# COMBINE-lab/salmon

Measured on NVIDIA H100. Metric: EM iters/s, higher is better.
Workload: dtype f64

## Files before the change

include/salmon_b200.h:

```cpp
#ifndef SALMON_B200_H
#define SALMON_B200_H

#include <stddef.h>
#include <stdint.h>

#ifdef __cplusplus
extern "C" {
#endif

#define SB_OK 0
#define SB_ERR_INVALID (-1)
#define SB_ERR_NO_DEVICE (-2)
#define SB_ERR_CUDA (-3)
#define SB_ERR_NOMEM (-4)
#define SB_ERR_NCCL (-5)
#define SB_ERR_STATE (-6)

int sb_version(void);
const char* sb_last_error(void);
int sb_device_count(void);

typedef struct sb_eq_csr {
  uint64_t n_classes;
  uint32_t n_txps;
// ... 341 lines not shown
                     sb_map_batch_stats* stats);

typedef struct sb_read_meta {
  const char* names;
  const uint64_t* name_off;
  const uint8_t* qual_left;
  const uint8_t* qual_right;
} sb_read_meta;
int64_t sb_reads_next_meta(sb_reads* r, uint32_t max_pairs, uint32_t stride, uint8_t* left, uint8_t* right,
                           uint32_t* len_left, uint32_t* len_right, int want_quals, sb_read_meta* meta);
typedef int (*sb_batch_meta_cb)(void* user, const uint8_t* left, const uint8_t* right, uint32_t n_pairs, uint32_t read_len,
                                const sb_read_meta* meta);
typedef void (*sb_names_cb)(void* user, const char* names, size_t len);
int sb_reads_bucketed_meta(sb_reads* rd, uint32_t min_len, uint32_t batch, uint32_t max_read_len, uint32_t threads,
                           uint32_t shard_index, uint32_t shard_count, int want_quals, sb_batch_meta_cb cb,
                           sb_names_cb too_short, void* user, sb_bucket_stats* stats);

int sb_em_debug_timeline(sb_em_ctx* ctx, uint64_t* out, uint32_t iteration);

int sb_em_set_option(sb_em_ctx* ctx, const char* key, int64_t value);

int sb_em_get_info(sb_em_ctx* ctx, const char* key, int64_t* value);

int sb_nccl_unique_id(void* out128);
int sb_em_comm_init(sb_em_ctx* ctx, int rank, int nranks, const void* unique_id128);
int sb_em_comm_destroy(sb_em_ctx* ctx);
int sb_em_peer_handle(sb_em_ctx* ctx, uint32_t max_txps, void* out64);
int sb_em_peer_open(sb_em_ctx* ctx, int rank, int nranks, const void* handles );

int sb_flush_l2(sb_em_ctx* ctx);

int sb_host_register(void* ptr, size_t bytes);
int sb_host_unregister(void* ptr);

#ifdef __cplusplus
}
#endif
#endif
```

salmon_b200/_capi.py:

```python
from __future__ import annotations

import ctypes as C
import os
from dataclasses import dataclass

import numpy as np

_HERE = os.path.dirname(os.path.abspath(__file__))
LIB_PATH = os.path.join(_HERE, "libsalmon_b200.so")

SB_OK = 0


class SalmonB200Error(RuntimeError):
    pass


class sb_eq_csr(C.Structure):
    _fields_ = [
        ("n_classes", C.c_uint64),
        ("n_txps", C.c_uint32),
        ("off", C.c_void_p),
        ("tids", C.c_void_p),
        ("weights", C.c_void_p),
# ... 152 lines not shown
    "sb_eq_file_read": (C.c_int, [C.c_char_p, C.POINTER(C.POINTER(sb_eq_file))]),
    "sb_eq_file_free": (None, [C.POINTER(sb_eq_file)]),
    "sb_bootstrap_writer_open": (_P, [C.c_char_p]),
    "sb_bootstrap_writer_write": (C.c_int, [_P, _P, C.c_uint32]),
    "sb_bootstrap_writer_close": (C.c_int64, [_P]),
    "sb_txome_read_fasta": (C.c_int, [C.c_char_p, C.c_uint32, C.c_int, C.c_char_p, C.c_int, C.c_int,
                                      C.POINTER(C.POINTER(sb_txome))]),
    "sb_txome_free": (None, [C.POINTER(sb_txome)]),
    "sb_version": (C.c_int, []),
    "sb_last_error": (C.c_char_p, []),
    "sb_device_count": (C.c_int, []),
    "sb_em_default_params": (None, [C.POINTER(sb_em_params)]),
    "sb_em_create": (_P, [C.c_int]),
    "sb_em_destroy": (None, [_P]),
    "sb_em_optimize": (C.c_int, [_P, C.POINTER(sb_eq_csr), C.POINTER(sb_em_params), _P, _P, _P, _P,
                                 C.POINTER(sb_em_stats)]),
    "sb_em_upload": (C.c_int, [_P, C.POINTER(sb_eq_csr), _P, _P, _P]),
    "sb_em_prepare": (C.c_int, [_P, C.POINTER(sb_em_params), C.POINTER(sb_em_stats)]),
    "sb_em_run": (C.c_int, [_P, C.POINTER(sb_em_stats)]),
    "sb_em_download": (C.c_int, [_P, _P, C.POINTER(sb_em_stats)]),
    "sb_em_get_combined": (C.c_int, [_P, _P, _P]),
    "sb_em_set_option": (C.c_int, [_P, C.c_char_p, C.c_int64]),
    "sb_em_get_info": (C.c_int, [_P, C.c_char_p, C.POINTER(C.c_int64)]),
    "sb_em_debug_timeline": (C.c_int, [_P, _P, C.c_uint32]),
    "sb_bootstrap": (C.c_int, [_P, C.POINTER(sb_em_params), C.c_double, C.c_uint32, C.c_uint64, _P, _P]),
    "sb_bootstrap_last_counts": (C.c_int, [_P, _P]),
    "sb_gibbs": (C.c_int, [_P, _P, C.c_int, C.c_int, C.c_double, C.c_uint32, C.c_uint32, C.c_int, C.c_double,
                           C.c_uint64, _P, _P]),
    "sb_gibbs_last_state": (C.c_int, [_P, _P, _P]),
    "sb_nccl_unique_id": (C.c_int, [_P]),
    "sb_em_comm_init": (C.c_int, [_P, C.c_int, C.c_int, _P]),
    "sb_em_comm_destroy": (C.c_int, [_P]),
    "sb_em_peer_handle": (C.c_int, [_P, C.c_uint32, _P]),
    "sb_em_peer_open": (C.c_int, [_P, C.c_int, C.c_int, _P]),
    "sb_flush_l2": (C.c_int, [_P]),
    "sb_index_build": (_P, [C.c_uint32, _P, _P, C.c_uint32]),
    "sb_index_free": (None, [_P]),
    "sb_index_set_meta": (C.c_int, [_P, _P, _P, C.c_uint32]),
    "sb_index_get_meta": (C.c_int, [_P, _P, _P, _P, _P, _P]),
    "sb_index_save": (C.c_int, [_P, C.c_char_p]),
    "sb_index_load": (_P, [C.c_char_p]),
    "sb_index_info": (C.c_int, [_P, _P]),
    "sb_index_host_arrays": (C.c_int, [_P, _P, _P, _P, _P, _P, _P]),
    "sb_map_default_params": (None, [C.POINTER(sb_map_params)]),
    "sb_map_mimic_bt2": (C.c_int, [C.POINTER(sb_map_params), C.c_int]),
    "sb_map_create": (_P, [_P, C.POINTER(sb_map_params), C.c_int, C.c_uint32, C.c_uint32]),
# ... 161 lines not shown
            raise SalmonB200Error("sb_em_create failed: " + self.lib.sb_last_error().decode())
        self._keep = None
        self.M = 0

    def close(self):
        if self.h:
            self.lib.sb_em_destroy(self.h)
            self.h = None

    def __del__(self):
        try:
            self.close()
        except Exception:
            pass

    def set_option(self, key: str, value: int):
        _check(self.lib.sb_em_set_option(self.h, key.encode(), int(value)), "sb_em_set_option")

    def info(self, key: str) -> int:
        v = C.c_int64(0)
        _check(self.lib.sb_em_get_info(self.h, key.encode(), C.byref(v)), "sb_em_get_info")
        return v.value

    @staticmethod
    def _txp_arrays(eq, projected, eff_len, unique):
        projected = np.ascontiguousarray(projected, dtype=np.float64)
        eff_len = np.ascontiguousarray(eff_len, dtype=np.float64)
        unique = np.ascontiguousarray(unique, dtype=np.uint64)
        assert projected.shape[0] == eff_len.shape[0] == unique.shape[0] == eq.n_txps
        return projected, eff_len, unique

    def optimize(self, eq: EqClasses, params: sb_em_params, projected, eff_len, unique):
        projected, eff_len, unique = self._txp_arrays(eq, projected, eff_len, unique)
        alpha = np.empty(eq.n_txps, dtype=np.float64)
        st = sb_em_stats()
        s = eq.as_struct()
        rc = _check(self.lib.sb_em_optimize(self.h, C.byref(s), C.byref(params), projected.ctypes.data,
                                            eff_len.ctypes.data, unique.ctypes.data, alpha.ctypes.data,
                                            C.byref(st)), "sb_em_optimize")
        self.M = eq.n_txps
        self._nnz = eq.nnz
        self._C = eq.n_classes
        return alpha, st, rc == 0

    def upload(self, eq: EqClasses, projected, eff_len, unique):
        projected, eff_len, unique = self._txp_arrays(eq, projected, eff_len, unique)
# ... 669 lines not shown
```

salmon_b200/csrc/em.cu:

```cuda
#include <cooperative_groups.h>
#include <cub/cub.cuh>
#include <float.h>
#include <math.h>
#include <stdarg.h>
#include <string.h>

#include <algorithm>
#include <string>
#include <vector>

#include "common.cuh"
#include "em_internal.h"

#include "em_kernels.cuh"

namespace sb {

static const void* const K_PERSISTENT[2] = {(const void*)k_em_persistent<false>, (const void*)k_em_persistent<true>};
static const void* const K_PERSISTENT_MGPU[2] = {(const void*)k_em_persistent_mgpu<false>,
                                                 (const void*)k_em_persistent_mgpu<true>};
static void (*const K_P1[2])(EmArgs) = {k_em_p1<false>, k_em_p1<true>};
static void (*const K_P2[2])(EmArgs, uint32_t) = {k_em_p2<false>, k_em_p2<true>};
static void (*const K_P2_PARTIAL[2])(EmArgs) = {k_em_p2_partial<false>, k_em_p2_partial<true>};

// ... 153 lines not shown
  const uint32_t t = rank_tid[rowperm[r]];
  row_tid[r] = t;
  tid_row[t] = r;
  r_prior[r] = prior[t];
  r_base[r] = base[t];
  r_alpha0[r] = alpha0[t];
}
__global__ void k_gather_csc(uint32_t nnz, const uint32_t* __restrict__ perm,
                             const uint32_t* __restrict__ ent_cls,
                             const double* __restrict__ m_w, uint32_t* __restrict__ t_idx,
                             double* __restrict__ t_w) {
  uint32_t k = blockIdx.x * blockDim.x + threadIdx.x;
  if (k >= nnz) return;
  uint32_t j = perm[k];
  t_idx[k] = ent_cls[j];
  t_w[k] = m_w[j];
}
__global__ void k_remap(uint32_t n, const uint32_t* __restrict__ src,
                        const uint32_t* __restrict__ map, uint32_t* __restrict__ dst) {
  uint32_t k = blockIdx.x * blockDim.x + threadIdx.x;
  if (k < n) dst[k] = map[src[k]];
}

__global__ void k_sell_widths(uint32_t n_rows, uint32_t n_slices, const uint32_t* __restrict__ rowperm,
                              const uint32_t* __restrict__ csr_off, const uint32_t* __restrict__ csr_idx,
                              uint16_t* __restrict__ len16, uint32_t* __restrict__ width,
                              uint32_t* __restrict__ sbase, uint32_t* __restrict__ counts) {
  const uint32_t s = blockIdx.x * (blockDim.x >> 5) + (threadIdx.x >> 5);
  if (s >= n_slices) return;
  const uint32_t lane = threadIdx.x & 31;
  const uint32_t row = s * 32 + lane;
  uint32_t len = 0, lo = 0xffffffffu, hi = 0;
  bool sell = false;
  if (row < n_rows) {
    const uint32_t cr = rowperm ? rowperm[row] : row;
    const uint32_t b = csr_off[cr];
    len = csr_off[cr + 1] - b;
    sell = len <= LMAX;
    if (!sell) {
      len16[row] = LEN_LONG;
      atomicAdd(&counts[0], 1u);
      len = 0;
    }
    for (uint32_t j = 0; j < len; ++j) {
      lo = min(lo, csr_idx[b + j]);
      hi = max(hi, csr_idx[b + j]);
// ... 11 lines not shown
    if (fallback) {
      atomicAdd(&counts[0], 1u);
      atomicAdd(&counts[2], 1u);
    }
  }
  if (lane == 0) {
    width[s] = fallback ? 0u : width_s;
    sbase[s] = hi >= lo ? lo : 0u;
  }
}
__global__ void k_sell_fill(uint32_t n_rows, uint32_t n_slices, const uint32_t* __restrict__ rowperm,
                            const uint32_t* __restrict__ csr_off, const uint32_t* __restrict__ csr_idx,
                            const double* __restrict__ csr_w, const uint32_t* __restrict__ slice_ptr,
                            const uint32_t* __restrict__ sbase, const uint16_t* __restrict__ len16,
                            uint16_t* __restrict__ s_idx, double* __restrict__ s_w,
                            uint32_t* __restrict__ long_rows, uint32_t* __restrict__ long_cursor) {
  const uint32_t s = blockIdx.x * (blockDim.x >> 5) + (threadIdx.x >> 5);
  if (s >= n_slices) return;
  const uint32_t lane = threadIdx.x & 31;
  const uint32_t row = s * 32 + lane;
  const size_t first = (size_t)slice_ptr[s] * 32;
  const uint32_t width = slice_ptr[s + 1] - slice_ptr[s];
  const uint32_t grouped = width & ~3u;
  auto pos = [&](uint32_t j) {
    return j < grouped ? first + (size_t)(j >> 2) * 128 + lane * 4 + (j & 3u) : first + (size_t)j * 32 + lane;
  };
  const uint32_t base = sbase[s];
  uint32_t n = 0;
  if (row < n_rows) {
    const uint32_t cr = rowperm ? rowperm[row] : row;
    const uint32_t b = csr_off[cr], e = csr_off[cr + 1];
    if (len16[row] == LEN_LONG) {
      const uint32_t pos = atomicAdd(long_cursor, 1u);
      long_rows[3 * pos] = row;
      long_rows[3 * pos + 1] = b;
      long_rows[3 * pos + 2] = e;
    } else {
      n = e - b;
      for (uint32_t j = 0; j < n; ++j) {
        s_idx[pos(j)] = (uint16_t)(csr_idx[b + j] - base);
        s_w[pos(j)] = csr_w[b + j];
      }
    }
  }
  for (uint32_t j = n; j < width; ++j) {
    s_idx[pos(j)] = IDX_PAD;
    s_w[pos(j)] = 0.0;
  }
}
__global__ void k_warp_ranges(uint32_t n_slices, const uint32_t* __restrict__ slice_ptr,
                              uint32_t overhead, uint32_t n_warps, uint32_t* __restrict__ warp_begin) {
  const uint32_t wid = blockIdx.x * blockDim.x + threadIdx.x;
  if (wid > n_warps) return;
  if (wid == n_warps || n_slices == 0) { warp_begin[wid] = n_slices; return; }
  const uint64_t total = (uint64_t)slice_ptr[n_slices] + (uint64_t)overhead * n_slices;
  const uint64_t target = total * wid / n_warps;
  uint32_t lo = 0, hi = n_slices;
  while (lo < hi) {
    uint32_t mid = (lo + hi) >> 1;
    uint64_t wk = (uint64_t)slice_ptr[mid] + (uint64_t)overhead * mid;
    if (wk >= target) hi = mid; else lo = mid + 1;
  }
  warp_begin[wid] = lo;
}

__global__ void k_sum1(uint32_t M, const double* __restrict__ a, const double* __restrict__ b,
                       const uint32_t* __restrict__ tid_row, int mode, double* __restrict__ out) {
  __shared__ double scratch[32];
  double acc = 0.0;
  for (uint32_t i = threadIdx.x; i < M; i += blockDim.x) {
    if (mode == 1 && tid_row[i] != 0xffffffffu) continue;
    acc += a[i] + b[i];
// ... 212 lines not shown
  else if (!strcmp(key, "sample_offset")) { c->sample_offset = (uint32_t)value; }
  else if (!strcmp(key, "rebalance")) { c->rebalance = (int)value; c->prepared = false; }
  else { set_error("unknown option '%s'", key); return SB_ERR_INVALID; }
  return SB_OK;
}

extern "C" int sb_em_get_info(sb_em_ctx* c, const char* key, int64_t* value) {
  if (!c || !key || !value) { set_error("null argument"); return SB_ERR_INVALID; }
  if (!c->prepared) { set_error("sb_em_get_info before sb_em_prepare"); return SB_ERR_STATE; }
  auto stream = [](const SellDev& m) { return (int64_t)m.n_cols * 32 * 10 + (int64_t)m.long_entries * 12; };
  if (!strcmp(key, "stream_bytes")) { *value = stream(c->cm) + stream(c->tm); return SB_OK; }
  if (!strcmp(key, "warps")) { *value = (int64_t)c->grid * (EM_THREADS / 32); return SB_OK; }
  if (!strcmp(key, "ring_cols")) { *value = (int64_t)EM_CH * EM_RING; return SB_OK; }
  const size_t n = strlen(key);
  const SellDev* m = nullptr;
  if (n > 3 && !strcmp(key + n - 3, "_cm")) m = &c->cm;
  else if (n > 3 && !strcmp(key + n - 3, "_tm")) m = &c->tm;
  const std::string k(key, m ? n - 3 : n);
  if (m && k == "stream_bytes") *value = stream(*m);
  else if (m && k == "sell_cols") *value = m->n_cols;
  else if (m && k == "long_rows") *value = m->n_long;
  else if (m && k == "long_entries") *value = (int64_t)m->long_entries;
  else if (m && k == "fallback_rows") *value = m->n_fallback;
  else { set_error("unknown info key '%s'", key); return SB_ERR_INVALID; }
  return SB_OK;
}

extern "C" int sb_em_upload(sb_em_ctx* c, const sb_eq_csr* eq, const double* projected,
                            const double* eff_len, const uint64_t* unique) {
  if (!c || !eq || !projected || !eff_len || !unique) { set_error("null argument"); return SB_ERR_INVALID; }
  if (eq->n_classes && (!eq->off || !eq->counts)) { set_error("null CSR arrays"); return SB_ERR_INVALID; }
  SB_CUDA(cudaSetDevice(c->device));
  const uint64_t C = eq->n_classes;
  const uint32_t M = eq->n_txps;
  const uint64_t nnz = C ? eq->off[C] : 0;
  if (M == 0) { set_error("no transcripts"); return SB_ERR_INVALID; }
  if (nnz >= 0xfffffff0ull || C >= 0xfffffff0ull) {
    set_error("eq-class table too large for 32-bit device offsets (nnz=%llu)", (unsigned long long)nnz);
    return SB_ERR_INVALID;
  }
  if (nnz && (!eq->tids || !eq->weights)) { set_error("null CSR arrays"); return SB_ERR_INVALID; }
  c->C = C; c->M = M; c->nnz = nnz;
  c->prepared = false;
  SB_TRY(dev_alloc(&c->d_off, C + 1));
  SB_TRY(dev_alloc(&c->d_tids, nnz));
  SB_TRY(dev_alloc(&c->d_aux, nnz));
  SB_TRY(dev_alloc(&c->d_counts, C));
// ... 100 lines not shown
  }
  m.n_block = 0;
  m.long_entries = 0;
  if (m.n_long > 0) {
    std::vector<uint32_t> h((size_t)3 * m.n_long);
    SB_CUDA(cudaMemcpyAsync(h.data(), m.long_rows, h.size() * 4, cudaMemcpyDeviceToHost, st));
    SB_CUDA(cudaStreamSynchronize(st));
    std::vector<uint32_t> ord(m.n_long);
    for (uint32_t i = 0; i < m.n_long; ++i) ord[i] = i;
    std::sort(ord.begin(), ord.end(), [&](uint32_t x, uint32_t y) {
      const uint32_t lx = h[3 * x + 2] - h[3 * x + 1], ly = h[3 * y + 2] - h[3 * y + 1];
      return lx != ly ? lx > ly : h[3 * x] < h[3 * y];
    });
    for (uint32_t i = 0; i < m.n_long; ++i) {
      if (h[3 * ord[i] + 2] - h[3 * ord[i] + 1] > LWARP) m.n_block = i + 1;
      m.long_entries += h[3 * i + 2] - h[3 * i + 1];
    }
    std::vector<uint32_t> h2(h.size());
    for (uint32_t i = 0; i < m.n_long; ++i)
      for (int k = 0; k < 3; ++k) h2[3 * i + k] = h[3 * ord[i] + k];
    SB_CUDA(cudaMemcpyAsync(m.long_rows, h2.data(), h2.size() * 4, cudaMemcpyHostToDevice, st));
    SB_CUDA(cudaStreamSynchronize(st));
  }
  k_warp_ranges<<<nblk(n_warps + 1, 256), 256, 0, st>>>(m.n_slices, m.slice_ptr, overhead, n_warps, m.warp_begin);
  c->launches++;
  return SB_OK;
}

static int em_rebalance(sb_em_ctx* c);

extern "C" int sb_em_prepare(sb_em_ctx* c, const sb_em_params* p, sb_em_stats* stats) {
  if (!c || !p) { set_error("null argument"); return SB_ERR_INVALID; }
  if (!c->uploaded) { set_error("sb_em_prepare before sb_em_upload"); return SB_ERR_STATE; }
  SB_CUDA(cudaSetDevice(c->device));
  cudaStream_t st = c->stream;
  c->params = *p;
  c->launches = 0;
  const uint64_t C = c->C;
  const uint32_t M = c->M;
  const uint64_t nnz = c->nnz;
  const bool row_space = c->nranks <= 1 && !c->fused_loopback;
  SB_CUDA(cudaEventRecord(c->ev[0], st));

  int occ = 0;
  for (int v = 0; v < 2; ++v) {
    SB_CUDA(cudaFuncSetAttribute(K_PERSISTENT[v], cudaFuncAttributeMaxDynamicSharedMemorySize, (int)EM_SMEM));
    SB_CUDA(cudaFuncSetAttribute((const void*)K_P1[v], cudaFuncAttributeMaxDynamicSharedMemorySize, (int)EM_SMEM));
    SB_CUDA(cudaFuncSetAttribute((const void*)K_P2[v], cudaFuncAttributeMaxDynamicSharedMemorySize, (int)EM_SMEM));
// ... 190 lines not shown
    stats->gpu_launches = prep_launches;
  }
  return SB_OK;
}

static Sell sell_view(const SellDev& m) {
  Sell s;
  s.slice_ptr = m.slice_ptr; s.base = m.base; s.len = m.len; s.idx = m.idx; s.w = m.w; s.warp_begin = m.warp_begin;
  s.long_rows = m.long_rows; s.csr_idx = m.csr_idx; s.csr_w = m.csr_w;
  s.n_rows = m.n_rows; s.n_slices = m.n_slices; s.n_long = m.n_long;
  s.n_block = m.n_block;
  s.zero = m.zero;
  return s;
}

static void fill_args(sb_em_ctx* c, EmArgs& A, bool row_space) {
  memset(&A, 0, sizeof(A));
  A.cm = sell_view(c->cm);
  A.tm = sell_view(c->tm);
  const bool ov = c->ov_active;
  A.c_cnt = (ov && c->ov_cnt) ? c->ov_cnt : c->d_cnt; A.scale = c->d_scale;
  if (row_space) {
    A.alpha = c->r_alpha; A.theta = c->r_theta; A.prior = c->r_prior;
    A.base = (ov && c->ov_base_row) ? c->ov_base_row : c->r_base;
    A.row_tid = nullptr;
  } else {
    A.alpha = c->d_alpha; A.theta = c->d_theta; A.prior = c->d_prior; A.base = c->d_base;
    A.row_tid = c->d_row_tid;
    A.tid_row = c->d_tid_row;
  }
  A.sum_partial = c->d_sum_partial;
  A.maxrel = (unsigned long long*)(c->d_scalars + 24);
  A.inactive_sum = ov ? c->ov_inactive_sum : c->inactive_sum;
  A.sum0 = ov ? c->ov_sum0 : c->sum0;
  A.min_eq_w = ov ? c->ov_min_eq_w : DBL_MIN;
  A.first_bias = ov ? 0.0 : (c->params.use_vbem ? 0.0 : 1.0);
  A.tol = c->params.tol; A.min_iter = c->params.min_iter; A.max_iter = c->params.max_iter;
  A.out = (uint32_t*)(c->d_scalars + 32);
  A.lq = (unsigned int*)(c->d_scalars + 44);
  A.dbg = c->dbg_enabled ? c->d_dbg : nullptr;
  A.dbg_it = c->dbg_it;
}

#include <dlfcn.h>
namespace {
struct NcclUid { char b[128]; };
// ... 524 lines not shown
```

salmon_b200/csrc/em_internal.h:

```cpp
#pragma once
#include <cuda_runtime.h>
#include <stdint.h>

#include <vector>

#include "../../include/salmon_b200.h"

namespace sb {

constexpr int SELL_GROUP = 1024;

struct SellDev {
  uint32_t n_rows = 0, n_slices = 0, n_cols = 0, n_long = 0, n_block = 0;
  uint32_t n_fallback = 0;
  uint64_t long_entries = 0;
  uint32_t zero = 0;
  uint32_t* slice_ptr = nullptr;
  uint32_t* width = nullptr;
  uint32_t* base = nullptr;
  uint16_t* len = nullptr;
  uint16_t* idx = nullptr;
  double* w = nullptr;
  uint32_t* warp_begin = nullptr;
  uint32_t* long_rows = nullptr;
  const uint32_t* csr_idx = nullptr;
  const double* csr_w = nullptr;
};

}

struct sb_em_ctx {
  int device = 0;
  int n_sm = 0;
  size_t l2_bytes = 0;
  cudaStream_t stream = nullptr;
  cudaEvent_t ev[4] = {nullptr, nullptr, nullptr, nullptr};

  int variant = 1;
// ... 103 lines not shown
```

salmon_b200/csrc/em_kernels.cuh:

```cuda
#pragma once
#include <cooperative_groups.h>
#include <float.h>

#include "common.cuh"
#include "em_math.h"

namespace sb {
namespace cg = cooperative_groups;

constexpr uint32_t LMAX = 96;
constexpr uint32_t LWARP = 2048;
constexpr int EM_THREADS = 256;
constexpr int EM_CH = 8;
constexpr int EM_RING = 4;
constexpr int EM_MIN_BLOCKS = 2;
constexpr double DIGAMMA_MIN = 1e-10;
constexpr double MIN_EQ_W = DBL_MIN;
constexpr double ALPHA_CHECK_CUTOFF = 1e-2;
constexpr uint16_t LEN_LONG = 0xFFFFu;
constexpr uint16_t IDX_PAD = 0xFFFFu;
constexpr uint32_t DBG_ACCUMULATE = 0xFFFFFFFFu;
constexpr uint32_t DBG_SLOTS = 16;

struct Sell {
  const uint32_t* slice_ptr;
  const uint32_t* base;
  const uint16_t* len;
  const uint16_t* idx;
  const double* w;
  const uint32_t* warp_begin;
  const uint32_t* long_rows;
  const uint32_t* csr_idx;
  const double* csr_w;
  uint32_t n_rows, n_slices, n_long;
  uint32_t n_block;
  uint32_t zero;
};

struct EmArgs {
  Sell cm;
  Sell tm;
  const double* c_cnt;
  double* scale;
  double* alpha; double* theta; const double* prior; const double* base;
  const uint32_t* row_tid;
  const uint32_t* tid_row;
  double* part_out;
  double* sum_partial;
  unsigned long long* maxrel;
  double inactive_sum; double sum0;
  double tol;
  double min_eq_w;
  double first_bias;
  uint32_t min_iter, max_iter;
  uint32_t* out;
  unsigned long long* dbg;
  uint32_t dbg_it;
  unsigned int* lq;
  unsigned char* const* peers;
  uint32_t rank, nranks, M;
  uint32_t push_pass;
  unsigned long long epoch0;
  uint32_t* xfail;
};

constexpr uint32_t XAUX = 1024;
struct XchgLayout {
  uint32_t M, G, S;
  __host__ __device__ XchgLayout(uint32_t m, uint32_t g) : M(m), G(g), S((m + g - 1) / g) {}
  __host__ __device__ size_t off_flags() const { return 0; }
  __host__ __device__ size_t off_theta() const { return 64 * 8; }
  __host__ __device__ size_t off_alpha() const { return off_theta() + ((size_t)M + 4) * 8; }
  __host__ __device__ size_t off_llth() const { return (off_alpha() + (size_t)M * 8 + 15) & ~(size_t)15; }
  __host__ __device__ size_t off_llaux() const { return off_llth() + (size_t)M * 16; }
  __host__ __device__ size_t off_llrecv() const { return off_llaux() + (size_t)G * XAUX * 2 * 16; }
  __host__ __device__ size_t bytes() const { return off_llrecv() + (size_t)G * S * 16; }
};

__device__ __forceinline__ unsigned long long gtime_ns() {
  unsigned long long t;
  asm volatile("mov.u64 %0, %%globaltimer;" : "=l"(t));
  return t;
}

constexpr double SUM_FIXED = 1048576.0;
struct P2Acc {
  long long isum;
  double maxrel;
};
__device__ __forceinline__ long long warp_sum_ll(long long v) {
#pragma unroll
  for (int o = 16; o > 0; o >>= 1) v += __shfl_xor_sync(0xffffffffu, v, o);
  return v;
}
__device__ __forceinline__ long long block_sum_ll(long long v, double* scratch) {
  const int lane = threadIdx.x & 31, wid = threadIdx.x >> 5;
  const int nw = (blockDim.x + 31) >> 5;
  v = warp_sum_ll(v);
  __syncthreads();
  if (lane == 0) scratch[wid] = __longlong_as_double(v);
  __syncthreads();
  long long r = (lane < nw) ? __double_as_longlong(scratch[lane]) : 0ll;
  return warp_sum_ll(r);
}

struct __align__(128) WarpRing {
  double w[EM_RING][EM_CH * 32];
  uint16_t idx[EM_RING][EM_CH * 32];
};
constexpr int EM_WARPS = EM_THREADS / 32;
constexpr size_t EM_SMEM = sizeof(WarpRing) * EM_WARPS + EM_WARPS * EM_RING * 8 + 40 * 8;
// ... 12 lines not shown
__device__ __forceinline__ void warp_setup(WarpCtx& W, unsigned char* smem) {
  const uint32_t wid = threadIdx.x >> 5;
  W.ring = reinterpret_cast<WarpRing*>(smem) + wid;
  W.bars = reinterpret_cast<uint64_t*>(smem + sizeof(WarpRing) * EM_WARPS) + wid * EM_RING;
  W.scratch = reinterpret_cast<double*>(smem + sizeof(WarpRing) * EM_WARPS + EM_WARPS * EM_RING * 8);
  W.phase_bits = 0;
  W.dbg = nullptr;
  W.dbg_acc = nullptr;
  W.t0 = 0;
  W.pol_stream = l2_policy_evict_first();
  if ((threadIdx.x & 31u) == 0) {
#pragma unroll
    for (int s = 0; s < EM_RING; ++s) mbar_init(&W.bars[s], 1);
    mbar_fence_init();
  }
  __syncthreads();
}

struct RowOps {
  double x0, x1, x2, x3;
  uint32_t len;
};
template <int PHASE>
__device__ __forceinline__ RowOps load_ops(const EmArgs& A, const Sell& S, uint32_t row) {
  RowOps o;
  o.x0 = o.x1 = o.x2 = o.x3 = 0.0;
  o.len = LEN_LONG;
  if (row < S.n_rows) {
    o.len = __ldg(&S.len[row]);
    if (PHASE == 1) {
      o.x0 = __ldg(&A.c_cnt[row]);
    } else if (PHASE == 2) {
      o.x0 = A.theta[row];
      o.x1 = __ldg(&A.prior[row]);
      o.x2 = __ldg(&A.base[row]);
      o.x3 = A.alpha[row];
    } else {
      const uint32_t t = __ldg(&A.row_tid[row]);
      o.x0 = A.theta[t];
      o.x2 = __ldg(&A.base[t]);
      o.x3 = __longlong_as_double((long long)t);
    }
  }
  return o;
}

template <bool VBEM>
__device__ __forceinline__ double theta_of(double na, double ap, double logNorm) {
  if (VBEM) return (ap > DIGAMMA_MIN) ? exp_digamma_shifted(ap, logNorm) : 0.0;
  return na;
}

template <int PHASE, bool VBEM, class Deliver>
__device__ __forceinline__ void row_finish(const EmArgs& A, uint32_t row, const RowOps& o, double acc,
                                           double logNorm, double bias, P2Acc& pa, Deliver&& deliver) {
  if (o.len == LEN_LONG) return;
  if (PHASE == 1) {
    A.scale[row] = (acc <= A.min_eq_w) ? 0.0 : o.x0 / acc;
  } else if (PHASE == 2) {
    const double th = o.x0, pr = o.x1;
    double na = o.x2 + bias;
    if (th > 0.0) na = fma(th, acc, na);
    if (na > ALPHA_CHECK_CUTOFF) pa.maxrel = fmax(pa.maxrel, fabs(o.x3 - na) / na);
    A.alpha[row] = na;
    const double ap = na + pr;
    pa.isum += __double2ll_rn(ap * SUM_FIXED);
    A.theta[row] = theta_of<VBEM>(na, ap, logNorm);
  } else {
    const uint32_t t = (uint32_t)__double_as_longlong(o.x3);
    double na = o.x2;
    if (o.x0 > 0.0) na = fma(o.x0, acc, na);
    deliver(t, na);
  }
}

struct WarpRange {
  uint32_t s0, s1, cbeg, cend;
};
__device__ __forceinline__ WarpRange load_range(const Sell& S, uint32_t gwarp) {
  WarpRange r;
  r.s0 = __ldg(&S.warp_begin[gwarp]);
  r.s1 = __ldg(&S.warp_begin[gwarp + 1]);
  r.cbeg = __ldg(&S.slice_ptr[r.s0]);
  r.cend = __ldg(&S.slice_ptr[r.s1]);
  return r;
}
__device__ __forceinline__ void ring_issue(const Sell& S, WarpCtx& W, const WarpRange& R, uint32_t k) {
// ... 68 lines not shown
  };
  struct Group {
    double g0, g1, g2, g3;
    double2 wa, wb;
  };
  auto group_load = [&](uint32_t c, uint32_t base) {
    const uint2 i2 = cols.idx4(c);
    Group q;
    q.g0 = gsrc[slot(base, i2.x & 0xFFFFu)];
    q.g1 = gsrc[slot(base, i2.x >> 16)];
    q.g2 = gsrc[slot(base, i2.y & 0xFFFFu)];
    q.g3 = gsrc[slot(base, i2.y >> 16)];
    q.wa = cols.w4(c, 0u);
    q.wb = cols.w4(c, 2u);
    return q;
  };
  auto group_fma = [&](double& acc, const Group& q) {
    fma1(acc, q.g0, q.wa.x); fma1(acc, q.g1, q.wa.y); fma1(acc, q.g2, q.wb.x); fma1(acc, q.g3, q.wb.y);
  };
  uint32_t sbase = s0;
  uint32_t sp = (s0 + lane < s1) ? __ldg(&S.slice_ptr[s0 + lane + 1]) : cend;
  uint32_t sb = (s0 + lane < s1) ? __ldg(&S.base[s0 + lane]) : 0u;
  uint32_t c = 0;
  RowOps ops_next = load_ops<PHASE>(A, S, s0 * 32u + lane);
  for (uint32_t s = s0; s < s1; ++s) {
    if (s - sbase == 32u) {
      sbase = s;
      sp = (s + lane < s1) ? __ldg(&S.slice_ptr[s + lane + 1]) : cend;
      sb = (s + lane < s1) ? __ldg(&S.base[s + lane]) : 0u;
    }
    const uint32_t slice_end = __shfl_sync(0xffffffffu, sp, (int)(s - sbase)) - cbeg;
    const uint32_t base = __shfl_sync(0xffffffffu, sb, (int)(s - sbase));
    uint32_t ng = (slice_end - c) >> 2;
    const uint32_t rem = (slice_end - c) & 3u;
    const RowOps ops = ops_next;
    if (s + 1u < s1) ops_next = load_ops<PHASE>(A, S, (s + 1u) * 32u + lane);
    if (slice_end == c) continue;
    double acc = 0.0;
    for (; ng >= 2; ng -= 2, c += 8) {
      cols.need(c, c + 8);
      const Group qa = group_load(c, base);
      const Group qb = group_load(c + 4, base);
      group_fma(acc, qa);
      group_fma(acc, qb);
    }
    if (ng) {
      cols.need(c, c + 4);
      group_fma(acc, group_load(c, base));
      c += 4;
    }
    if (rem) {
      cols.need(c, c + rem);
      const double g0 = gsrc[slot(base, cols.idx1(c))];
      if (rem == 1) {
        fma1(acc, g0, cols.w1(c));
      } else if (rem == 2) {
        const double g1 = gsrc[slot(base, cols.idx1(c + 1))];
        fma1(acc, g0, cols.w1(c)); fma1(acc, g1, cols.w1(c + 1));
      } else {
// ... 32 lines not shown
    const uint32_t r = __ldg(&S.long_rows[3 * li]);
    const uint32_t b = __ldg(&S.long_rows[3 * li + 1]);
    const uint32_t e = __ldg(&S.long_rows[3 * li + 2]);
    double a0 = 0.0, a1 = 0.0;
    uint32_t k = b + threadIdx.x;
    for (; k + EM_THREADS < e; k += 2 * EM_THREADS) {
      const uint32_t i0 = __ldg(&S.csr_idx[k]), i1 = __ldg(&S.csr_idx[k + EM_THREADS]);
      double v0 = gsrc[i0] * __ldg(&S.csr_w[k]);
      double v1 = gsrc[i1] * __ldg(&S.csr_w[k + EM_THREADS]);
      if (GUARD) {
        if (isnan(v0)) v0 = 0.0;
        if (isnan(v1)) v1 = 0.0;
      }
      a0 += v0;
      a1 += v1;
    }
    if (k < e) {
      double v = gsrc[__ldg(&S.csr_idx[k])] * __ldg(&S.csr_w[k]);
      if (GUARD && isnan(v)) v = 0.0;
      a0 += v;
    }
    const double acc = block_reduce<false>(a0 + a1, W.scratch);
    if (threadIdx.x == 0) {
      RowOps o = load_ops<PHASE>(A, S, r);
      o.len = 0;
      row_finish<PHASE, VBEM>(A, r, o, acc, logNorm, bias, pa, deliver);
    }
    __syncthreads();
  }
  {
    const uint32_t gw = bid * EM_WARPS + (threadIdx.x >> 5);
    const uint32_t nw = nblk * EM_WARPS;
    const uint32_t n_mid = S.n_long - S.n_block;
    unsigned int* queue = A.lq + ((PHASE == 1) ? 0 : 1);
    uint32_t cnt = 0, myrow = 0xffffffffu;
    double myacc = 0.0;
    auto flush = [&]() {
      if (myrow != 0xffffffffu) {
        RowOps o = load_ops<PHASE>(A, S, myrow);
        o.len = 0;
        row_finish<PHASE, VBEM>(A, myrow, o, myacc, logNorm, bias, pa, deliver);
      }
      myrow = 0xffffffffu;
      cnt = 0;
    };
    auto claim = [&]() -> uint32_t {
      uint32_t q = 0;
      if (lane == 0) q = atomicAdd(queue, 1u);
      return q;
    };
    uint32_t q_next;
    if (DYNQ) q_next = n_mid ? claim() : 0u; else q_next = gw;
    unsigned long long* const qs = (dbg && lane == 0) ? dbg + (PHASE == 1 ? 9 : 11) : nullptr;
    for (;;) {
      const uint32_t q = DYNQ ? __shfl_sync(0xffffffffu, q_next, 0) : q_next;
      if (q >= n_mid) break;
      if (DYNQ) q_next = claim(); else q_next = q + nw;
      const uint32_t li = S.n_block + q;
      const uint32_t r = __ldg(&S.long_rows[3 * li]);
      const uint32_t b = __ldg(&S.long_rows[3 * li + 1]);
      const uint32_t e = __ldg(&S.long_rows[3 * li + 2]);
      double a0 = 0.0, a1 = 0.0, a2 = 0.0, a3 = 0.0;
// ... 93 lines not shown
  W.dbg_acc = nullptr; \
  if (dbg_acc && (threadIdx.x & 31u) == 0) A.dbg[(size_t)gwarp * DBG_SLOTS + (slot)] += gtime_ns() - var;

template <bool VBEM>
__global__ void __launch_bounds__(EM_THREADS, EM_MIN_BLOCKS) k_em_persistent(const __grid_constant__ EmArgs A) {
  extern __shared__ __align__(128) unsigned char smem[];
  WarpCtx W;
  warp_setup(W, smem);
  double* scratch = W.scratch;
  cg::grid_group grid = cg::this_grid();
  const uint32_t bid = blockIdx.x, nblk = gridDim.x;
  const uint32_t gwarp = bid * (EM_THREADS / 32) + (threadIdx.x >> 5);
  const WarpRange R1 = load_range(A.cm, gwarp);
  const WarpRange R2 = load_range(A.tm, gwarp);
  uint32_t it = 0;
  bool converged = false;
  double logNorm = VBEM ? digamma_pos(A.sum0) : 0.0;
  ring_prefetch(A.cm, W, R1);
  while (it < A.min_iter || (it < A.max_iter && !converged)) {
    const uint32_t par = it & 1u;
    const bool dbg_acc = A.dbg && A.dbg_it == DBG_ACCUMULATE && it > 0;
    if (bid == 0 && threadIdx.x == 0) A.maxrel[par] = 0ull;
    if (VBEM && it > 0) lag_lognorm_warp0(A, par, nblk, scratch);
    P2Acc pa{0ll, 0.0};
    SB_DBG(0)
    SB_ACC_BEGIN(t1, 3)
    W.dbg = (A.dbg && it == A.dbg_it) ? &A.dbg[(size_t)gwarp * DBG_SLOTS] : nullptr;
    run_phase<1, VBEM, true>(A, W, R1, bid, nblk, 0.0, 0.0, pa, [&] { ring_prefetch(A.tm, W, R2); }, NoDeliver{});
    SB_ACC_END(t1, 0)
    SB_DBG(1)
    grid.sync();
    SB_DBG(2)
    if (bid == 0 && threadIdx.x == 0) A.lq[0] = 0u;
    if (VBEM && it > 0) logNorm = scratch[33];
    const double bias = (it == 0) ? A.first_bias : 0.0;
    SB_DBG(3)
    SB_ACC_BEGIN(t2, 4)
    run_phase<2, VBEM, true>(A, W, R2, bid, nblk, logNorm, bias, pa, [&] { ring_prefetch(A.cm, W, R1); }, NoDeliver{});
    W.dbg = nullptr;
    SB_ACC_END(t2, 1)
    SB_DBG(4)
    p2_finish(A, scratch, pa, par);
    SB_DBG(5)
    grid.sync();
    SB_DBG(6)
    if (bid == 0 && threadIdx.x == 0) A.lq[1] = 0u;
    if (dbg_acc && (threadIdx.x & 31u) == 0) A.dbg[(size_t)gwarp * DBG_SLOTS + 2] += 1ull;
// ... 90 lines not shown
  cg::grid_group grid = cg::this_grid();
  const uint32_t bid = blockIdx.x, nblk = gridDim.x;
  const uint32_t gwarp = bid * (EM_THREADS / 32) + (threadIdx.x >> 5);
  const uint32_t gtid = bid * EM_THREADS + threadIdx.x, gthreads = nblk * EM_THREADS;
  const WarpRange R1 = load_range(A.cm, gwarp);
  const WarpRange R2 = load_range(A.tm, gwarp);
  const uint32_t M = A.M, G = A.nranks;
  const XchgLayout X(M, G);
  const uint32_t S = X.S, lo = min(A.rank * S, M), hi = min(lo + S, M);
  unsigned char* const own = A.peers[A.rank];
  const uint4* my_recv = reinterpret_cast<const uint4*>(own + X.off_llrecv());
  const uint4* my_llth = reinterpret_cast<const uint4*>(own + X.off_llth());
  const uint4* my_aux = reinterpret_cast<const uint4*>(own + X.off_llaux());
  double* theta = A.theta;
  uint32_t it = 0;
  bool converged = false;
  double logNorm = VBEM ? digamma_pos(A.sum0) : 0.0;
  ring_prefetch(A.cm, W, R1);
  while (it < A.min_iter || (it < A.max_iter && !converged)) {
    const uint32_t par = it & 1u;
    const uint32_t epoch = (uint32_t)(A.epoch0 + it + 1ull);
    const DeliverPush push{A.peers, X.off_llrecv(), S, A.rank, epoch};
    const bool dbg_acc = A.dbg && A.dbg_it == DBG_ACCUMULATE && it > 0;
    P2Acc pa{0ll, 0.0};
    SB_DBG(0)
    SB_ACC_BEGIN(t1, 3)
    run_phase<1, VBEM, true>(A, W, R1, bid, nblk, 0.0, 0.0, pa, [&] { ring_prefetch(A.tm, W, R2); }, NoDeliver{});
    SB_ACC_END(t1, 0)
    SB_DBG(1)
    grid.sync();
    SB_DBG(2)
    if (bid == 0 && threadIdx.x == 0) A.lq[0] = 0u;
    SB_ACC_BEGIN(t2, 4)
    if (A.push_pass) {
      run_phase<3, VBEM, true>(A, W, R2, bid, nblk, 0.0, 0.0, pa, [&] { ring_prefetch(A.cm, W, R1); },
                               DeliverLocal{A.part_out});
      SB_ACC_END(t2, 1)
      SB_DBG(3)
      __threadfence();
      grid.sync();
      if (bid == 0 && threadIdx.x == 0) A.lq[1] = 0u;
      for (uint32_t t = gtid; t < M; t += gthreads) push(t, __ldcg(&A.part_out[t]));
    } else {
      for (uint32_t t = gtid; t < M; t += gthreads)
        if (__ldg(&A.tid_row[t]) == 0xffffffffu) push(t, __ldg(&A.base[t]));
      run_phase<3, VBEM, true>(A, W, R2, bid, nblk, 0.0, 0.0, pa, [&] { ring_prefetch(A.cm, W, R1); }, push);
      SB_ACC_END(t2, 1)
// ... 89 lines not shown
    SB_DBG(7)
    if (dbg_acc && (threadIdx.x & 31u) == 0) A.dbg[(size_t)gwarp * DBG_SLOTS + 2] += 1ull;
    ++it;
  }
  for (uint32_t t = lo + gtid; t < hi; t += gthreads) {
    const double a = A.alpha[t];
    for (uint32_t q = 0; q < G; ++q) st_relaxed_sys_f64(reinterpret_cast<double*>(A.peers[q] + X.off_alpha()) + t, a);
  }
  xgpu_barrier(grid, A, A.epoch0 + it + 1ull);
  if (bid == 0 && threadIdx.x == 0) {
    A.out[0] = it;
    A.out[1] = converged ? 1u : 0u;
    A.out[2] = (it - 1) & 1u;
    A.out[3] = it + 2u;
  }
  ring_drain(W, R1);
}

template <bool VBEM>
__global__ void __launch_bounds__(EM_THREADS, EM_MIN_BLOCKS) k_em_p1(const __grid_constant__ EmArgs A) {
  extern __shared__ __align__(128) unsigned char smem[];
  WarpCtx W;
  warp_setup(W, smem);
  P2Acc pa{0ll, 0.0};
  const WarpRange R = load_range(A.cm, blockIdx.x * (EM_THREADS / 32) + (threadIdx.x >> 5));
  ring_prefetch(A.cm, W, R);
  run_phase<1, VBEM, false>(A, W, R, blockIdx.x, gridDim.x, 0.0, 0.0, pa, Nothing{}, NoDeliver{});
}
template <bool VBEM>
__global__ void __launch_bounds__(EM_THREADS, EM_MIN_BLOCKS) k_em_p2(const __grid_constant__ EmArgs A, uint32_t it) {
  extern __shared__ __align__(128) unsigned char smem[];
  WarpCtx W;
  warp_setup(W, smem);
  double* scratch = W.scratch;
  const uint32_t par = it & 1u;
  double logNorm = 0.0;
  if (VBEM) {
    if (it == 0) {
      logNorm = digamma_pos(A.sum0);
    } else {
      lag_lognorm_warp0(A, par, gridDim.x, scratch);
      __syncthreads();
      logNorm = scratch[33];
    }
  }
  const double bias = (it == 0) ? A.first_bias : 0.0;
  P2Acc pa{0ll, 0.0};
  const WarpRange R = load_range(A.tm, blockIdx.x * (EM_THREADS / 32) + (threadIdx.x >> 5));
  ring_prefetch(A.tm, W, R);
  run_phase<2, VBEM, false>(A, W, R, blockIdx.x, gridDim.x, logNorm, bias, pa, Nothing{}, NoDeliver{});
  p2_finish(A, scratch, pa, par);
}
template <bool VBEM>
__global__ void __launch_bounds__(EM_THREADS, EM_MIN_BLOCKS) k_em_p2_partial(const __grid_constant__ EmArgs A) {
  extern __shared__ __align__(128) unsigned char smem[];
  WarpCtx W;
  warp_setup(W, smem);
  P2Acc pa{0ll, 0.0};
  const WarpRange R = load_range(A.tm, blockIdx.x * (EM_THREADS / 32) + (threadIdx.x >> 5));
  ring_prefetch(A.tm, W, R);
  run_phase<3, VBEM, false>(A, W, R, blockIdx.x, gridDim.x, 0.0, 0.0, pa, Nothing{}, DeliverLocal{A.part_out});
}

}
```

Baseline: 26710.

## Skip alpha reads/writes before min_iter and broadcast uniform prior

```diff
diff --git a/include/salmon_b200.h b/include/salmon_b200.h
--- a/include/salmon_b200.h
+++ b/include/salmon_b200.h
@@ -387,6 +387,9 @@
 
 int sb_em_get_info(sb_em_ctx* ctx, const char* key, int64_t* value);
 
+int sb_em_get_layout(sb_em_ctx* ctx, int which, uint32_t* slice_ptr, uint32_t* base, uint16_t* idx,
+                     uint32_t* long_rows, uint32_t* csr_idx);
+
 int sb_nccl_unique_id(void* out128);
 int sb_em_comm_init(sb_em_ctx* ctx, int rank, int nranks, const void* unique_id128);
 int sb_em_comm_destroy(sb_em_ctx* ctx);
diff --git a/salmon_b200/_capi.py b/salmon_b200/_capi.py
--- a/salmon_b200/_capi.py
+++ b/salmon_b200/_capi.py
@@ -198,6 +198,7 @@
     "sb_em_get_combined": (C.c_int, [_P, _P, _P]),
     "sb_em_set_option": (C.c_int, [_P, C.c_char_p, C.c_int64]),
     "sb_em_get_info": (C.c_int, [_P, C.c_char_p, C.POINTER(C.c_int64)]),
+    "sb_em_get_layout": (C.c_int, [_P, C.c_int, _P, _P, _P, _P, _P]),
     "sb_em_debug_timeline": (C.c_int, [_P, _P, C.c_uint32]),
     "sb_bootstrap": (C.c_int, [_P, C.POINTER(sb_em_params), C.c_double, C.c_uint32, C.c_uint64, _P, _P]),
     "sb_bootstrap_last_counts": (C.c_int, [_P, _P]),
@@ -405,6 +406,16 @@
         _check(self.lib.sb_em_get_info(self.h, key.encode(), C.byref(v)), "sb_em_get_info")
         return v.value
 
+    def layout(self, which: str, rows: int, nnz_multi: int) -> dict:
+        ns = (rows + 31) // 32
+        out = {"slice_ptr": np.zeros(ns + 1, np.uint32), "base": np.zeros(max(ns, 1), np.uint32),
+               "idx": np.zeros(max(self.info("sell_cols_" + which) * 32, 1), np.uint16),
+               "long_rows": np.zeros(max(3 * self.info("long_rows_" + which), 1), np.uint32),
+               "csr_idx": np.zeros(max(nnz_multi, 1), np.uint32)}
+        _check(self.lib.sb_em_get_layout(self.h, 1 if which == "tm" else 0, *(a.ctypes.data for a in out.values())),
+               "sb_em_get_layout")
+        return out
+
     @staticmethod
     def _txp_arrays(eq, projected, eff_len, unique):
         projected = np.ascontiguousarray(projected, dtype=np.float64)
diff --git a/salmon_b200/csrc/em.cu b/salmon_b200/csrc/em.cu
--- a/salmon_b200/csrc/em.cu
+++ b/salmon_b200/csrc/em.cu
@@ -199,6 +199,9 @@
   if (k < n) dst[k] = map[src[k]];
 }
 
+__device__ __forceinline__ size_t sell_entry(size_t first, uint32_t grouped, uint32_t lane, uint32_t j) {
+  return j < grouped ? first + (size_t)(j >> 2) * 128 + lane * 4 + (j & 3u) : first + (size_t)j * 32 + lane;
+}
 __global__ void k_sell_widths(uint32_t n_rows, uint32_t n_slices, const uint32_t* __restrict__ rowperm,
                               const uint32_t* __restrict__ csr_off, const uint32_t* __restrict__ csr_idx,
                               uint16_t* __restrict__ len16, uint32_t* __restrict__ width,
@@ -256,9 +259,7 @@
   const size_t first = (size_t)slice_ptr[s] * 32;
   const uint32_t width = slice_ptr[s + 1] - slice_ptr[s];
   const uint32_t grouped = width & ~3u;
-  auto pos = [&](uint32_t j) {
-    return j < grouped ? first + (size_t)(j >> 2) * 128 + lane * 4 + (j & 3u) : first + (size_t)j * 32 + lane;
-  };
+  auto pos = [&](uint32_t j) { return sell_entry(first, grouped, lane, j); };
   const uint32_t base = sbase[s];
   uint32_t n = 0;
   if (row < n_rows) {
@@ -282,6 +283,37 @@
     s_w[pos(j)] = 0.0;
   }
 }
+__device__ __forceinline__ uint32_t warp_distinct(uint32_t line, bool valid) {
+  const unsigned peers = __match_any_sync(0xffffffffu, valid ? line : 0xFFFFFFFFu);
+  return __popc(__ballot_sync(0xffffffffu, valid && (threadIdx.x & 31u) == (uint32_t)(__ffs(peers) - 1)));
+}
+__global__ void k_lines_sell(uint32_t n_slices, const uint32_t* __restrict__ slice_ptr,
+                             const uint32_t* __restrict__ sbase, const uint16_t* __restrict__ s_idx, uint32_t zero,
+                             unsigned long long* __restrict__ out) {
+  const uint32_t s = blockIdx.x * (blockDim.x >> 5) + (threadIdx.x >> 5);
+  if (s >= n_slices) return;
+  const uint32_t lane = threadIdx.x & 31;
+  const size_t first = (size_t)slice_ptr[s] * 32;
+  const uint32_t width = slice_ptr[s + 1] - slice_ptr[s];
+  const uint32_t base = sbase[s];
+  unsigned long long n = 0;
+  for (uint32_t j = 0; j < width; ++j) {
+    const uint16_t u = s_idx[sell_entry(first, width & ~3u, lane, j)];
+    n += warp_distinct((u == IDX_PAD ? zero : base + u) >> 4, true);
+  }
+  if (lane == 0 && n) atomicAdd(out, n);
+}
+__global__ void k_lines_long(uint32_t n_long, const uint32_t* __restrict__ long_rows,
+                             const uint32_t* __restrict__ csr_idx, unsigned long long* __restrict__ out) {
+  const uint32_t li = blockIdx.x * (blockDim.x >> 5) + (threadIdx.x >> 5);
+  if (li >= n_long) return;
+  const uint32_t lane = threadIdx.x & 31;
+  const uint32_t b = long_rows[3 * li + 1], e = long_rows[3 * li + 2];
+  unsigned long long n = 0;
+  for (uint32_t k = b; k < e; k += 32) n += warp_distinct(k + lane < e ? csr_idx[k + lane] >> 4 : 0u, k + lane < e);
+  if (lane == 0 && n) atomicAdd(out, n);
+}
+
 __global__ void k_warp_ranges(uint32_t n_slices, const uint32_t* __restrict__ slice_ptr,
                               uint32_t overhead, uint32_t n_warps, uint32_t* __restrict__ warp_begin) {
   const uint32_t wid = blockIdx.x * blockDim.x + threadIdx.x;
@@ -540,7 +572,22 @@
   else if (m && k == "long_rows") *value = m->n_long;
   else if (m && k == "long_entries") *value = (int64_t)m->long_entries;
   else if (m && k == "fallback_rows") *value = m->n_fallback;
+  else if (m && k == "gather_lines") *value = (int64_t)m->gather_lines;
   else { set_error("unknown info key '%s'", key); return SB_ERR_INVALID; }
+  return SB_OK;
+}
+
+extern "C" int sb_em_get_layout(sb_em_ctx* c, int which, uint32_t* slice_ptr, uint32_t* base, uint16_t* idx,
+                                uint32_t* long_rows, uint32_t* csr_idx) {
+  if (!c || (which != 0 && which != 1)) { set_error("bad argument"); return SB_ERR_INVALID; }
+  if (!c->prepared) { set_error("sb_em_get_layout before sb_em_prepare"); return SB_ERR_STATE; }
+  SB_CUDA(cudaSetDevice(c->device));
+  const SellDev& m = which ? c->tm : c->cm;
+  if (slice_ptr) SB_CUDA(cudaMemcpy(slice_ptr, m.slice_ptr, ((size_t)m.n_slices + 1) * 4, cudaMemcpyDeviceToHost));
+  if (base && m.n_slices) SB_CUDA(cudaMemcpy(base, m.base, (size_t)m.n_slices * 4, cudaMemcpyDeviceToHost));
+  if (idx && m.n_cols) SB_CUDA(cudaMemcpy(idx, m.idx, (size_t)m.n_cols * 32 * 2, cudaMemcpyDeviceToHost));
+  if (long_rows && m.n_long) SB_CUDA(cudaMemcpy(long_rows, m.long_rows, (size_t)m.n_long * 12, cudaMemcpyDeviceToHost));
+  if (csr_idx && c->nnzm) SB_CUDA(cudaMemcpy(csr_idx, m.csr_idx, (size_t)c->nnzm * 4, cudaMemcpyDeviceToHost));
   return SB_OK;
 }
 
@@ -687,8 +734,14 @@
     SB_CUDA(cudaMemcpyAsync(m.long_rows, h2.data(), h2.size() * 4, cudaMemcpyHostToDevice, st));
     SB_CUDA(cudaStreamSynchronize(st));
   }
+  unsigned long long* d_lines = (unsigned long long*)(c->d_scalars + 12);
+  SB_CUDA(cudaMemsetAsync(d_lines, 0, 8, st));
+  if (m.n_slices) k_lines_sell<<<nblk(m.n_slices, 8), 256, 0, st>>>(m.n_slices, m.slice_ptr, m.base, m.idx, m.zero, d_lines);
+  if (m.n_long) k_lines_long<<<nblk(m.n_long, 8), 256, 0, st>>>(m.n_long, m.long_rows, m.csr_idx, d_lines);
   k_warp_ranges<<<nblk(n_warps + 1, 256), 256, 0, st>>>(m.n_slices, m.slice_ptr, overhead, n_warps, m.warp_begin);
-  c->launches++;
+  c->launches += 1 + (m.n_slices ? 1 : 0) + (m.n_long ? 1 : 0);
+  SB_CUDA(cudaMemcpyAsync(&m.gather_lines, d_lines, 8, cudaMemcpyDeviceToHost, st));
+  SB_CUDA(cudaStreamSynchronize(st));
   return SB_OK;
 }
 
@@ -925,6 +978,7 @@
   A.c_cnt = (ov && c->ov_cnt) ? c->ov_cnt : c->d_cnt; A.scale = c->d_scale;
   if (row_space) {
     A.alpha = c->r_alpha; A.theta = c->r_theta; A.prior = c->r_prior;
+    A.prior_all = c->params.per_txp_prior ? c->params.vb_prior : 0.0;
     A.base = (ov && c->ov_base_row) ? c->ov_base_row : c->r_base;
     A.row_tid = nullptr;
   } else {
diff --git a/salmon_b200/csrc/em_internal.h b/salmon_b200/csrc/em_internal.h
--- a/salmon_b200/csrc/em_internal.h
+++ b/salmon_b200/csrc/em_internal.h
@@ -14,6 +14,7 @@
   uint32_t n_rows = 0, n_slices = 0, n_cols = 0, n_long = 0, n_block = 0;
   uint32_t n_fallback = 0;
   uint64_t long_entries = 0;
+  uint64_t gather_lines = 0;
   uint32_t zero = 0;
   uint32_t* slice_ptr = nullptr;
   uint32_t* width = nullptr;
diff --git a/salmon_b200/csrc/em_kernels.cuh b/salmon_b200/csrc/em_kernels.cuh
--- a/salmon_b200/csrc/em_kernels.cuh
+++ b/salmon_b200/csrc/em_kernels.cuh
@@ -43,6 +43,7 @@
   const double* c_cnt;
   double* scale;
   double* alpha; double* theta; const double* prior; const double* base;
+  double prior_all;
   const uint32_t* row_tid;
   const uint32_t* tid_row;
   double* part_out;
@@ -87,6 +88,8 @@
 struct P2Acc {
   long long isum;
   double maxrel;
+  bool rel;
+  bool keep;
 };
 __device__ __forceinline__ long long warp_sum_ll(long long v) {
 #pragma unroll
@@ -145,7 +148,7 @@
   uint32_t len;
 };
 template <int PHASE>
-__device__ __forceinline__ RowOps load_ops(const EmArgs& A, const Sell& S, uint32_t row) {
+__device__ __forceinline__ RowOps load_ops(const EmArgs& A, const Sell& S, uint32_t row, bool rel) {
   RowOps o;
   o.x0 = o.x1 = o.x2 = o.x3 = 0.0;
   o.len = LEN_LONG;
@@ -155,9 +158,9 @@
       o.x0 = __ldg(&A.c_cnt[row]);
     } else if (PHASE == 2) {
       o.x0 = A.theta[row];
-      o.x1 = __ldg(&A.prior[row]);
+      o.x1 = A.prior_all > 0.0 ? A.prior_all : __ldg(&A.prior[row]);
       o.x2 = __ldg(&A.base[row]);
-      o.x3 = A.alpha[row];
+      o.x3 = rel ? A.alpha[row] : 0.0;
     } else {
       const uint32_t t = __ldg(&A.row_tid[row]);
       o.x0 = A.theta[t];
@@ -184,8 +187,8 @@
     const double th = o.x0, pr = o.x1;
     double na = o.x2 + bias;
     if (th > 0.0) na = fma(th, acc, na);
-    if (na > ALPHA_CHECK_CUTOFF) pa.maxrel = fmax(pa.maxrel, fabs(o.x3 - na) / na);
-    A.alpha[row] = na;
+    if (pa.rel && na > ALPHA_CHECK_CUTOFF) pa.maxrel = fmax(pa.maxrel, fabs(o.x3 - na) / na);
+    if (pa.keep) A.alpha[row] = na;
     const double ap = na + pr;
     pa.isum += __double2ll_rn(ap * SUM_FIXED);
     A.theta[row] = theta_of<VBEM>(na, ap, logNorm);
@@ -300,7 +303,7 @@
   uint32_t sp = (s0 + lane < s1) ? __ldg(&S.slice_ptr[s0 + lane + 1]) : cend;
   uint32_t sb = (s0 + lane < s1) ? __ldg(&S.base[s0 + lane]) : 0u;
   uint32_t c = 0;
-  RowOps ops_next = load_ops<PHASE>(A, S, s0 * 32u + lane);
+  RowOps ops_next = load_ops<PHASE>(A, S, s0 * 32u + lane, pa.rel);
   for (uint32_t s = s0; s < s1; ++s) {
     if (s - sbase == 32u) {
       sbase = s;
@@ -312,7 +315,7 @@
     uint32_t ng = (slice_end - c) >> 2;
     const uint32_t rem = (slice_end - c) & 3u;
     const RowOps ops = ops_next;
-    if (s + 1u < s1) ops_next = load_ops<PHASE>(A, S, (s + 1u) * 32u + lane);
+    if (s + 1u < s1) ops_next = load_ops<PHASE>(A, S, (s + 1u) * 32u + lane, pa.rel);
     if (slice_end == c) continue;
     double acc = 0.0;
     for (; ng >= 2; ng -= 2, c += 8) {
@@ -391,7 +394,7 @@
     }
     const double acc = block_reduce<false>(a0 + a1, W.scratch);
     if (threadIdx.x == 0) {
-      RowOps o = load_ops<PHASE>(A, S, r);
+      RowOps o = load_ops<PHASE>(A, S, r, pa.rel);
       o.len = 0;
       row_finish<PHASE, VBEM>(A, r, o, acc, logNorm, bias, pa, deliver);
     }
@@ -406,7 +409,7 @@
     double myacc = 0.0;
     auto flush = [&]() {
       if (myrow != 0xffffffffu) {
-        RowOps o = load_ops<PHASE>(A, S, myrow);
+        RowOps o = load_ops<PHASE>(A, S, myrow, pa.rel);
         o.len = 0;
         row_finish<PHASE, VBEM>(A, myrow, o, myacc, logNorm, bias, pa, deliver);
       }
@@ -546,7 +549,7 @@
     const bool dbg_acc = A.dbg && A.dbg_it == DBG_ACCUMULATE && it > 0;
     if (bid == 0 && threadIdx.x == 0) A.maxrel[par] = 0ull;
     if (VBEM && it > 0) lag_lognorm_warp0(A, par, nblk, scratch);
-    P2Acc pa{0ll, 0.0};
+    P2Acc pa{0ll, 0.0, it + 1 >= A.min_iter, it + 2 >= A.min_iter};
     SB_DBG(0)
     SB_ACC_BEGIN(t1, 3)
     W.dbg = (A.dbg && it == A.dbg_it) ? &A.dbg[(size_t)gwarp * DBG_SLOTS] : nullptr;
@@ -683,7 +686,7 @@
     const uint32_t epoch = (uint32_t)(A.epoch0 + it + 1ull);
     const DeliverPush push{A.peers, X.off_llrecv(), S, A.rank, epoch};
     const bool dbg_acc = A.dbg && A.dbg_it == DBG_ACCUMULATE && it > 0;
-    P2Acc pa{0ll, 0.0};
+    P2Acc pa{0ll, 0.0, true, true};
     SB_DBG(0)
     SB_ACC_BEGIN(t1, 3)
     run_phase<1, VBEM, true>(A, W, R1, bid, nblk, 0.0, 0.0, pa, [&] { ring_prefetch(A.tm, W, R2); }, NoDeliver{});
@@ -819,7 +822,7 @@
   extern __shared__ __align__(128) unsigned char smem[];
   WarpCtx W;
   warp_setup(W, smem);
-  P2Acc pa{0ll, 0.0};
+  P2Acc pa{0ll, 0.0, true, true};
   const WarpRange R = load_range(A.cm, blockIdx.x * (EM_THREADS / 32) + (threadIdx.x >> 5));
   ring_prefetch(A.cm, W, R);
   run_phase<1, VBEM, false>(A, W, R, blockIdx.x, gridDim.x, 0.0, 0.0, pa, Nothing{}, NoDeliver{});
@@ -842,7 +845,7 @@
     }
   }
   const double bias = (it == 0) ? A.first_bias : 0.0;
-  P2Acc pa{0ll, 0.0};
+  P2Acc pa{0ll, 0.0, it + 1 >= A.min_iter, it + 2 >= A.min_iter};
   const WarpRange R = load_range(A.tm, blockIdx.x * (EM_THREADS / 32) + (threadIdx.x >> 5));
   ring_prefetch(A.tm, W, R);
   run_phase<2, VBEM, false>(A, W, R, blockIdx.x, gridDim.x, logNorm, bias, pa, Nothing{}, NoDeliver{});
@@ -853,7 +856,7 @@
   extern __shared__ __align__(128) unsigned char smem[];
   WarpCtx W;
   warp_setup(W, smem);
-  P2Acc pa{0ll, 0.0};
+  P2Acc pa{0ll, 0.0, true, true};
   const WarpRange R = load_range(A.tm, blockIdx.x * (EM_THREADS / 32) + (threadIdx.x >> 5));
   ring_prefetch(A.tm, W, R);
   run_phase<3, VBEM, false>(A, W, R, blockIdx.x, gridDim.x, 0.0, 0.0, pa, Nothing{}, DeliverLocal{A.part_out});
```

After: 27560, median of 6. 1.03x the previous value.
